# ColumbiaDVMM/ColumbiaImageSearch

Measured on AMD Instinct MI355X. Metric: queries/sec @ recall@10 on 10M LOPQ index, higher is better.
Workload: dtype f64

## Files before the change

### __graft_entry__.py

```python
import os
import subprocess
import sys

REPO = os.path.dirname(os.path.abspath(__file__))
if REPO not in sys.path:
    sys.path.insert(0, REPO)


def build():
    csrc = os.path.join(REPO, "columbiaimagesearch_amd", "csrc")
    subprocess.check_call(["make", "-C", csrc, "-j4"])
    from columbiaimagesearch_amd import _lib
    import columbiaimagesearch_amd.lopq
    assert _lib.lib().cis_version() >= 100


def smoke():
    import numpy as np
    sys.path.insert(0, os.path.join(REPO, "tests"))
    from conftest import load_golden
    from test_lopq_hip_parity import hip_model
    from columbiaimagesearch_amd.lopq import LOPQSearcherHIP
    from oracle import lopq_oracle as O
    z, X, Q = load_golden("c2")
    m = hip_model(z)
    n = 20000
    coarse, fine = m.predict_batch(X[:n])
    om = O.OracleModel.from_npz(z)
    oc, of = O.compute_codes(om, X[:n])
    assert (coarse == oc).all() and (fine == of).all(), "encode parity"
    s = LOPQSearcherHIP(m)
    s.add_codes_array(coarse, fine)
    oi = O.OracleCSRIndex(om, oc, of)
    want = [oi.search(Q[qi], quota=1000, limit=100) for qi in range(16)]
    for route, prefilter in (("float32-prefilter scan", True), ("all-candidates select", False)):
        s.set_scan_mode(prefilter_only=prefilter)
        r = s.search_batch(Q[:16], quota=1000, limit=100)
        for qi in range(16):
            ids, dists, visited = want[qi]
            k = int(r["n_found"][qi])
            assert k == len(ids) and visited == int(r["visited"][qi]), "visited / count parity (%s)" % route
            assert (r["ids"][qi, :k] == ids).all(), "candidate id parity (%s)" % route
            assert np.allclose(r["dists"][qi, :k], dists, rtol=1e-9, atol=1e-12), "distance parity (%s)" % route
    print("smoke ok: %d vectors encoded, 16 queries searched on both routes, parity with oracle" % n)


if __name__ == "__main__":
    build()
    if len(sys.argv) > 1 and sys.argv[1] == "smoke":
        smoke()
```

### columbiaimagesearch_amd/csrc/lopq_search.hip

```cpp
#include "lopq_batch.h"

template <typename CT>
__global__ __launch_bounds__(256) void k_tables(const CT* __restrict__ X , const CT* __restrict__ Cs,
                                                const double* __restrict__ Rt, const double* __restrict__ mus,
                                                const double* __restrict__ subs, const TabDesc* __restrict__ tabs,
                                                int V, int h, int w, int nf, int K, int D,
                                                double* __restrict__ T , PwProg prog_w,
                                                double* __restrict__ px_out ,
                                                const int* __restrict__ tab_order, int first) {
    extern __shared__ __attribute__((aligned(16))) char smem[];
    double* v = reinterpret_cast<double*>(smem);
    double* px = v + h;
    const int tab = tab_order ? tab_order[first + blockIdx.x] : first + (int)blockIdx.x;
    const TabDesc td = tabs[tab];
    const int s = td.split, c = td.cluster;
    const CT* x = X + (int64_t)td.q * D + s * h;
    const CT* Cc = Cs + ((int64_t)s * V + c) * h;
    const double* mu = mus + ((int64_t)s * V + c) * h;
    const double* R = Rt + ((int64_t)s * V + c) * h * h;
    for (int k = threadIdx.x; k < h; k += blockDim.x) {
        const CT res = x[k] - Cc[k];
        v[k] = (double)res - mu[k];
    }
    __syncthreads();
// ... 958 lines not shown
    constexpr double EPS32 = 2.0 * M * 5.9604644775390625e-8;
    const double infl = 1.0 + 2.0 * EPS32;
    CodeWords<M> dup[G];
    bool has_dup[G];
    bool any_dup = false;
#pragma unroll
    for (int g = 0; g < G; ++g) { cnt[g] = 0; has_dup[g] = false; dup[g] = CodeWords<M>(); }
#ifndef CIS_SCAN_PLAIN_LOADS
    __amdgpu_buffer_rsrc_t rs;
    {
        const uint64_t cbase = (uint64_t)(uintptr_t)(codes + start * M);
        const uint32_t blo = (uint32_t)__builtin_amdgcn_readfirstlane((int)(uint32_t)cbase);
        const uint32_t bhi = (uint32_t)__builtin_amdgcn_readfirstlane((int)(uint32_t)(cbase >> 32));
        const int nbytes = __builtin_amdgcn_readfirstlane(len * M);
        rs = __builtin_amdgcn_make_buffer_rsrc((void*)(uintptr_t)(((uint64_t)bhi << 32) | blo), 0, nbytes, 0x00020000);
    }
#define CIS_LOAD_CODE(p) load_code_buf<M>(rs, (p))
#else
#define CIS_LOAD_CODE(p) load_code<M>(codes, start + ((p) < len ? (p) : len - 1))
#endif
    CodeWords<M> nxt[U];
    if (w < nit) {
#pragma unroll
        for (int u = 0; u < U; ++u) nxt[u] = CIS_LOAD_CODE(w * 64 * U + u * 64 + lane);
    }
    for (int iter = w; iter < nit; iter += NW) {
        const int base = iter * 64 * U;
        CodeWords<M> cur[U];
#pragma unroll
        for (int u = 0; u < U; ++u) cur[u] = nxt[u];
        if (iter + NW < nit) {
#pragma unroll
            for (int u = 0; u < U; ++u) nxt[u] = CIS_LOAD_CODE((iter + NW) * 64 * U + u * 64 + lane);
        }
        float d[U][G];
#ifndef CIS_SCAN_NO_PIPELINE
        if constexpr (G >= 2) {
            typename AdcVec<G>::type fbuf[2][M];
            adc32_issue<M, G>(cur[0], tab, rc, fbuf[0]);
#pragma unroll
            for (int u = 0; u < U; ++u) {
                if (u + 1 < U) adc32_issue<M, G>(cur[u + 1], tab, rc, fbuf[(u + 1) & 1]);
                __builtin_amdgcn_sched_barrier(0);
                adc32_reduce<M, G>(fbuf[u & 1], d[u]);
                __builtin_amdgcn_sched_barrier(0);
            }
        } else
#endif
        {
#pragma unroll
            for (int u = 0; u < U; ++u) adc32g<M, G>(cur[u], tab, rc, d[u]);
        }
        if (base + 64 * U > len) {
            const float QNAN = __int_as_float(0x7fc00000);
#pragma unroll
            for (int u = 0; u < U; ++u)
#pragma unroll
                for (int g = 0; g < G; ++g) d[u][g] = (base + u * 64 + lane < len) ? d[u][g] : QNAN;
        }
        unsigned long long pm[U][G];
        unsigned long long any = 0ull;
#pragma unroll
        for (int g = 0; g < G; ++g) {
            float thrm = block_bound_f32(&sh[g]) * margin;
#ifdef CIS_PROBE_HOTLOOP
            thrm = (margin > 100.f) ? thrm : -1.0f;
#endif
#pragma unroll
            for (int u = 0; u < U; ++u) {
                pm[u][g] = __ballot(d[u][g] <= thrm);
                any |= pm[u][g];
            }
        }
        if (any_dup) {
            any = 0ull;
#pragma unroll
            for (int g = 0; g < G; ++g) {
                const unsigned long long dup_on = has_dup[g] ? ~0ull : 0ull;
#pragma unroll
                for (int u = 0; u < U; ++u) {
                    bool same = true;
#pragma unroll
                    for (int i = 0; i < (M + 3) / 4; ++i) same = same && (cur[u].w[i] == dup[g].w[i]);
                    pm[u][g] &= ~(__ballot(same) & dup_on);
                    any |= pm[u][g];
                }
            }
        }
        if (any == 0ull) continue;
        const long long clk_s0 = CIS_CLK();
        ++n_slow;
#pragma unroll
        for (int g = 0; g < G; ++g) {
            if (g >= ng) break;
            uint64_t* rk = rk_all + (g * NW + w) * R;
            uint64_t* tr = tr_all + (g * NW + w) * 64;
            uint32_t* rp = nullptr;
            int ntot = 0;
#pragma unroll
            for (int u = 0; u < U; ++u) ntot += __popcll(pm[u][g]);
            if (ntot == 0) continue;
            if (cnt[g] + ntot <= R) {
                const int trash = (int)(tr - rk) + lane;
                int c = cnt[g];
#pragma unroll
                for (int u = 0; u < U; ++u) {
                    const unsigned long long m = pm[u][g];
                    const int idx = __builtin_amdgcn_mbcnt_hi((unsigned)(m >> 32), __builtin_amdgcn_mbcnt_lo((unsigned)m, c));
                    int sel;
                    asm("v_cndmask_b32_e64 %0, %1, %2, %3" : "=v"(sel) : "v"(trash), "v"(idx), "s"(m));
                    rk[sel] = ((uint64_t)__float_as_uint(d[u][g]) << 32) | (uint32_t)(base + u * 64 + lane);
                    c += __popcll(m);
                }
                cnt[g] = c;
                n_app += ntot;
                continue;
            }
            int u0 = 0;
            while (true) {
                bool full = false;
#pragma unroll
                for (int u = 0; u < U; ++u) {
                    const unsigned long long m = pm[u][g];
                    if (u < u0 || full || m == 0ull) continue;
                    const int n = __popcll(m);
                    if (cnt[g] + n > R) {
                        full = true;
                        u0 = u;
                        continue;
                    }
                    const int idx = cnt[g] + __builtin_amdgcn_mbcnt_hi((unsigned)(m >> 32), __builtin_amdgcn_mbcnt_lo((unsigned)m, 0));
                    if ((m >> lane) & 1ull) rk[idx] = ((uint64_t)__float_as_uint(d[u][g]) << 32) | (uint32_t)(base + u * 64 + lane);
                    cnt[g] += n;
                    n_app += n;
                    u0 = u + 1;
                }
                if (!full) break;
                const long long clk_c0 = CIS_CLK();
                int c2 = wave_compact_approx<NR, NW>(rk, cnt[g], L, Lw, R - 64, margin, infl, &sh[g], w);
                if (c2 < 0) {
                    uint32_t dp = 0xffffffffu;
                    const long long clk_e0 = CIS_CLK();
                    c2 = wave_compact_exact<M, NR, NW, false>(rk, rp, cnt[g], L, Lw, &sh[g], w, codes, start, K, T + (int64_t)it_tab0[g] * nf * K,
                                                                  T + (int64_t)it_tab1[g] * nf * K, dp);
                    clk_exact += CIS_CLK() - clk_e0;
                    dp = (uint32_t)__builtin_amdgcn_readfirstlane((int)dp);
                    if (dp != 0xffffffffu) {
                        dup[g] = load_code<M>(codes, start + (int64_t)dp);
                        has_dup[g] = true;
                        any_dup = true;
                    }
                }
                cnt[g] = c2;
                clk_comp += CIS_CLK() - clk_c0;
                const float thrm = block_bound_f32(&sh[g]) * margin;
                const unsigned long long dup_on = has_dup[g] ? ~0ull : 0ull;
#pragma unroll
                for (int u = 0; u < U; ++u) {
                    bool same = true;
#pragma unroll
                    for (int i = 0; i < (M + 3) / 4; ++i) same = same && (cur[u].w[i] == dup[g].w[i]);
                    pm[u][g] &= __ballot(d[u][g] <= thrm) & ~(__ballot(same) & dup_on);
                }
            }
        }
        clk_slow += CIS_CLK() - clk_s0;
    }
    const long long clk_loop_end = CIS_CLK();
    (void)clk_loop_end;
#pragma unroll
    for (int g = 0; g < G; ++g) {
        if (g >= ng) break;
        uint64_t* rk = rk_all + (g * NW + w) * R;
        if (cnt[g] > 0) cnt[g] = wave_compact_approx<NR, NW>(rk, cnt[g], L, Lw, NR * 64, margin, infl, &sh[g], w);
    }
    clk_final = CIS_CLK() - clk_loop_end;
    __syncthreads();
#pragma unroll
    for (int g = 0; g < G; ++g) {
        if (g >= ng) break;
        uint64_t* rk = rk_all + (g * NW + w) * R;
        cnt[g] = wave_filter_approx<NR, NW>(rk, cnt[g], margin, &sh[g]);
        if (lane == 0) sh[g].wcnt[w] = cnt[g];
#ifndef CIS_SCAN_NO_QBOUND
        if (tid == 0) {
            const uint64_t b = block_bound_u64<NW>(&sh[g]);
            if (b < sh[g].ext) atomicMin(&qbound[it_q[g]], (unsigned long long)b);
        }
#endif
    }
    const long long clk_exact_end = CIS_CLK();
    (void)clk_exact_end;
    __syncthreads();
#pragma unroll
    for (int g = 0; g < G; ++g) {
        if (g >= ng) break;
        const uint64_t* rk = rk_all + (g * NW + w) * R;
        int off = 0, total = 0;
#pragma unroll
        for (int i = 0; i < NW; ++i) {
            const int c = sh[g].wcnt[i];
            off += (i < w) ? c : 0;
            total += c;
        }
        uint64_t* out = item_surv + (int64_t)item_idx[g] * S + off;
        for (int e = lane; e < cnt[g]; e += 64) out[e] = rk[e];
        if (tid == 0) item_n[item_idx[g]] = total;
    }
#ifdef CIS_SCAN_COUNTERS
    CIS_CTR(3, n_slow);
    CIS_CTR(8, clk_exact);
    CIS_CTR(10, clk_exact_end - clk_loop_end);
    CIS_CTR(11, clk_tab_end - clk_begin);
    CIS_CTR(9, clk_final);
    CIS_CTR(4, n_app);
    CIS_CTR(5, clk_comp);
    CIS_CTR(6, clk_slow - clk_comp);
    CIS_CTR(7, CIS_CLK() - clk_begin);
    CIS_CTR(2, clk_loop_end - clk_begin);
#endif
}

template <int M, int NR, int U, int G, int NW>
__global__ __launch_bounds__(NW * 64) __attribute__((amdgpu_waves_per_eu(NR == 16 ? 2 : (G == 4 ? 2 : ((M == 16 && G == 2) ? 3 : 4)), 4))) void k_adc_scan2(const WorkItem* __restrict__ items, const int* __restrict__ slots,
                                                       const int* __restrict__ n_slots_ptr, const double* __restrict__ T,
                                                       const float* __restrict__ T32,
                                                       const uint8_t* __restrict__ codes, const int64_t* __restrict__ ids,
                                                       int K, int L, int S, float margin,
                                                       int* __restrict__ queue_ctr ,
                                                       uint64_t* __restrict__ item_surv, int* __restrict__ item_n,
                                                       unsigned long long* __restrict__ qbound ) {
    extern __shared__ __attribute__((aligned(16))) char smem[];
    constexpr int R = NR * 64 - 8;
    int* s_next = reinterpret_cast<int*>(smem + (size_t)K * M * G * 4 + (size_t)G * NW * (R + 64) * 8 + G * sizeof(ScanShared));
    const int* qs = n_slots_ptr + 8;
    const int home = blockIdx.x & 7;
    for (int a = 0; a < 8; ++a) {
        const int x = (home + a) & 7;
        const int qstart = qs[x];
        const int count = qs[x + 1] - qstart;
        while (true) {
            __syncthreads();
            if (threadIdx.x == 0) *s_next = atomicAdd(&queue_ctr[x], 1);
            __syncthreads();
            const int j = __builtin_amdgcn_readfirstlane(*s_next);
            if (j >= count) break;
            const int slot = qstart + j;
            int idx[G];
            int ng = 0;
            bool same = true;
#pragma unroll
            for (int g = 0; g < G; ++g) {
                idx[g] = slots[slot * G + g];
                if (idx[g] >= 0) {
                    ng = g + 1;
                    same = same && items[idx[g]].start == items[idx[0]].start && items[idx[g]].len == items[idx[0]].len;
                } else {
                    idx[g] = idx[0];
                }
            }
            if constexpr (G >= 2) {
                if (!same) {
                    for (int g2 = 0; g2 < ng; ++g2) {
                        int oi[G];
#pragma unroll
                        for (int g = 0; g < G; ++g) {
                            oi[g] = idx[0];
#pragma unroll
                            for (int gg = 1; gg < G; ++gg)
                                if (gg == g2) oi[g] = idx[gg];
                        }
                        if (g2 > 0) __syncthreads();
                        scan2_group<M, NR, U, G, NW>(items, oi, 1, T, T32, codes, ids, K, L, S, margin, item_surv, item_n, qbound, smem);
                    }
                    continue;
                }
            }
            scan2_group<M, NR, U, G, NW>(items, idx, ng, T, T32, codes, ids, K, L, S, margin, item_surv, item_n, qbound, smem);
        }
    }
}

template <int CAPM>
__global__ __launch_bounds__(256) void k_merge_items(const cis_hit* __restrict__ item_hits, const int* __restrict__ item_n,
                                                     const int64_t* __restrict__ item_off, int limit, int S,
                                                     cis_hit* __restrict__ out_hits, int64_t* __restrict__ out_ids,
                                                     double* __restrict__ out_dists, int* __restrict__ out_n,
                                                     int32_t* __restrict__ out_cells, uint32_t* __restrict__ out_pos) {
    extern __shared__ __attribute__((aligned(16))) char smem[];
    uint64_t* ka = reinterpret_cast<uint64_t*>(smem);
    uint64_t* kb = ka + CAPM;
    int64_t* pay = reinterpret_cast<int64_t*>(kb + CAPM);
    int* s_n = reinterpret_cast<int*>(pay + CAPM);
    const int q = blockIdx.x;
    const int64_t a = item_off[q], b = item_off[q + 1];
    const int64_t o = (int64_t)q * limit;
    merge_lists<CAPM>(item_hits, item_n, a, (int)(b - a), (int64_t)S, S, limit, ka, kb, pay, s_n,
                      out_hits ? out_hits + o : nullptr, out_ids ? out_ids + o : nullptr,
                      out_dists ? out_dists + o : nullptr, out_n ? out_n + q : nullptr,
                      out_cells ? out_cells + o : nullptr, out_pos ? out_pos + o : nullptr);
}


static __device__ __forceinline__ void wave_bitonic_lds(uint64_t* ka, uint64_t* kb, int N) {
    const int lane = threadIdx.x & 63;
    for (int k = 2; k <= N; k <<= 1) {
        for (int j = k >> 1; j > 0; j >>= 1) {
            for (int t = lane; t < (N >> 1); t += 64) {
                const int i = ((t & ~(j - 1)) << 1) | (t & (j - 1));
                const int p = i + j;
                const bool asc = ((i & k) == 0);
                const uint64_t a0 = ka[i], b0 = kb[i], a1 = ka[p], b1 = kb[p];
                const bool gt = (a0 > a1) || (a0 == a1 && b0 > b1);
                if (gt == asc) { ka[i] = a1; kb[i] = b1; ka[p] = a0; kb[p] = b0; }
            }
            wave_lds_sync();
        }
    }
}

template <int CAPM, int MT , int NEMAX >
#ifndef CIS_MERGE_WPE
#define CIS_MERGE_WPE 4
#endif
__global__ __launch_bounds__(256) __attribute__((amdgpu_waves_per_eu((MT == 16 || MT == 0) ? 2 : CIS_MERGE_WPE, 8)))
void k_merge_survivors(const uint64_t* __restrict__ surv ,
                                                         const int* __restrict__ item_n, const int64_t* __restrict__ item_off,
                                                         const WorkItem* __restrict__ items, const double* __restrict__ T,
                                                         const uint8_t* __restrict__ codes, const int64_t* __restrict__ ids,
                                                         int nq, int M, int K, int limit, int S,
                                                         cis_hit* __restrict__ out_hits, int64_t* __restrict__ out_ids,
                                                         double* __restrict__ out_dists, int* __restrict__ out_n,
                                                         int32_t* __restrict__ out_cells, uint32_t* __restrict__ out_pos,
                                                         const PlanOut* __restrict__ plan, int32_t* __restrict__ out_visited,
                                                         const float* __restrict__ item_slack ) {
    extern __shared__ __attribute__((aligned(16))) char smem[];
    const int lane = threadIdx.x & 63, wq = threadIdx.x >> 6;
    const int q = blockIdx.x * 4 + wq;
    if (q >= nq) return;
    if (lane == 0 && out_visited) out_visited[q] = plan[q].visited;
    uint64_t* ka = reinterpret_cast<uint64_t*>(smem) + (size_t)wq * 2 * CAPM;
    uint64_t* kb = ka + CAPM;
    const int64_t first = item_off[q];
    const int n_lists = (int)(item_off[q + 1] - first);
    const int nf = M / 2;
    int have = 0, l = 0, e = 0, total = 0;
    bool done_fast = false;
    if constexpr (MT != 0) {
        int cntl[4] = {0, 0, 0, 0}, n_total = 0;
        if (n_lists <= 4) {
#pragma unroll
            for (int i = 0; i < 4; ++i) {
                if (i < n_lists) cntl[i] = item_n[first + i];
                n_total += cntl[i];
            }
        }
        auto fast = [&](auto ne_tag) -> bool {
            constexpr int NE = decltype(ne_tag)::value;
            uint32_t hi[NE], pp[NE];
            int li[NE];
            bool valid[NE];
            uint32_t mn = 0xffffffffu, mx = 0u;
            uint64_t ent[NE];
            float ubv[NE];
#pragma unroll
            for (int i = 0; i < NE; ++i) {
                const int x = lane + 64 * i;
                valid[i] = x < n_total;
                int lst = 0, off = x;
#pragma unroll
                for (int j = 0; j < 3; ++j)
                    if (lst == j && off >= cntl[j]) { off -= cntl[j]; lst = j + 1; }
                li[i] = lst;
                ent[i] = surv[valid[i] ? (first + lst) * (int64_t)S + off : first * (int64_t)S];
            }
            if (item_slack) {
#pragma unroll
                for (int i = 0; i < NE; ++i) ubv[i] = item_slack[2 * (first + (valid[i] ? li[i] : 0)) + 1];
            }
#pragma unroll
            for (int i = 0; i < NE; ++i) {
                hi[i] = valid[i] ? (uint32_t)(ent[i] >> 32) : 0xffffffffu;
                pp[i] = valid[i] ? (uint32_t)ent[i] : 0xffffffffu;
                if (item_slack && valid[i])
                    hi[i] = __float_as_uint(__double2float_ru((double)(hi[i] + (uint32_t)MT) * (double)ubv[i]));
                mn = (valid[i] && hi[i] < mn) ? hi[i] : mn;
                mx = (valid[i] && hi[i] > mx) ? hi[i] : mx;
            }
            uint32_t thr = 0xffffffffu;
            float vub = __int_as_float(0x7f800000);
            float sl[4] = {0.f, 0.f, 0.f, 0.f};
            if (n_total > limit) {
                wave_minmax_step<1>(mn, mx); wave_minmax_step<2>(mn, mx); wave_minmax_step<4>(mn, mx);
                wave_minmax_step<8>(mn, mx); wave_minmax_step<16>(mn, mx); wave_minmax_step<32>(mn, mx);
                mn = (uint32_t)__builtin_amdgcn_readfirstlane((int)mn);
                mx = (uint32_t)__builtin_amdgcn_readfirstlane((int)mx);
                const uint32_t v = wave_kth_bisect<NE>(hi, valid, mn, mx, limit);
                if (item_slack) {
                    vub = __uint_as_float(v);
#pragma unroll
                    for (int i = 0; i < 4; ++i) sl[i] = (i < n_lists) ? item_slack[2 * (first + i)] : 0.f;
                } else {
                    const float margin = 1.0f + 3.0f * (2.0f * (float)MT * 5.9604645e-8f);
                    thr = __float_as_uint(__double2float_ru((double)__uint_as_float(v) * (double)margin));
                }
            }
            int kept = 0;
            int idx[NE];
            bool keep[NE];
#pragma unroll
            for (int i = 0; i < NE; ++i) {
                keep[i] = valid[i] && hi[i] <= thr;
                if (item_slack) {
                    const float s_i = li[i] == 0 ? sl[0] : (li[i] == 1 ? sl[1] : (li[i] == 2 ? sl[2] : sl[3]));
                    keep[i] = valid[i] && ((double)__uint_as_float(hi[i]) - (double)s_i <= (double)vub);
                }
                const unsigned long long m = __ballot(keep[i]);
                idx[i] = kept + __builtin_amdgcn_mbcnt_hi((unsigned)(m >> 32), __builtin_amdgcn_mbcnt_lo((unsigned)m, 0));
                kept += __popcll(m);
            }
            if (kept > CAPM) return false;
            WorkItem its[4];
#pragma unroll
            for (int i = 0; i < 4; ++i) its[i] = items[first + (i < n_lists ? i : 0)];
#pragma unroll
            for (int i0 = 0; i0 < NE; i0 += 4) {
                int64_t startv[4];
                const double* t0v[4];
                const double* t1v[4];
                uint32_t rankv[4], pos0v[4];
#pragma unroll
                for (int i = 0; i < 4; ++i) {
                    WorkItem it = its[0];
#pragma unroll
                    for (int j = 1; j < 4; ++j)
                        if (li[i0 + i] == j) it = its[j];
                    startv[i] = it.start; rankv[i] = (uint32_t)it.rank; pos0v[i] = (uint32_t)it.pos0;
                    t0v[i] = T + (int64_t)it.tab0 * nf * K;
                    t1v[i] = T + (int64_t)it.tab1 * nf * K;
                }
                CodeWords<MT> cw[4];
#pragma unroll
                for (int i = 0; i < 4; ++i) cw[i] = load_code<MT>(codes, startv[i] + (keep[i0 + i] ? pp[i0 + i] : 0u));
                double dd[4];
#pragma unroll
                for (int i = 0; i < 4; ++i) dd[i] = adc64_words<MT>(cw[i].w, K, t0v[i], t1v[i]);
#pragma unroll
                for (int i = 0; i < 4; ++i) {
                    if (keep[i0 + i]) {
                        ka[idx[i0 + i]] = (uint64_t)__double_as_longlong(dd[i]);
                        kb[idx[i0 + i]] = ((uint64_t)rankv[i] << 32) | (uint32_t)(pos0v[i] + pp[i0 + i]);
                    }
                }
            }
            int ns = 64;
            while (ns < kept) ns <<= 1;
            for (int x = kept + lane; x < ns; x += 64) { ka[x] = ~0ull; kb[x] = ~0ull; }
            wave_lds_sync();
            wave_bitonic_lds(ka, kb, ns);
            total = kept;
            return true;
        };
        if (n_lists >= 1 && n_lists <= 4) {
            if (n_total <= 256) done_fast = fast(std::integral_constant<int, 4>());
            else if (NEMAX >= 8 && n_total <= 512) {
                if constexpr (NEMAX >= 8) done_fast = fast(std::integral_constant<int, 8>());
            }
        }
    }
    while (!done_fast) {
        int n = have;
        int room = CAPM - have;
        while (l < n_lists && room > 0) {
            const int valid = item_n[first + l];
            const int take = (valid - e < room) ? (valid - e) : room;
            if (take > 0) {
                const WorkItem it = items[first + l];
                const double* t0 = T + (int64_t)it.tab0 * nf * K;
                const double* t1 = T + (int64_t)it.tab1 * nf * K;
                const uint64_t* src = surv + (first + l) * (int64_t)S + e;
                if constexpr (MT == 0) {
                    for (int x = lane; x < take; x += 64) {
                        const uint32_t p = (uint32_t)src[x];
                        ka[n + x] = (uint64_t)__double_as_longlong(adc64_global(codes, it.start + p, M, K, t0, t1));
                        kb[n + x] = ((uint64_t)(uint32_t)it.rank << 32) | (uint32_t)(it.pos0 + (int)p);
                    }
                } else {
                    for (int x0 = 0; x0 < take; x0 += 256) {
                        uint32_t p[4];
                        bool on[4];
#pragma unroll
                        for (int i = 0; i < 4; ++i) {
                            const int x = x0 + i * 64 + lane;
                            on[i] = x < take;
                            p[i] = on[i] ? (uint32_t)src[x] : 0u;
                        }
                        CodeWords<MT> cw[4];
#pragma unroll
                        for (int i = 0; i < 4; ++i) cw[i] = load_code<MT>(codes, it.start + p[i]);
                        double dd[4];
#pragma unroll
                        for (int i = 0; i < 4; ++i) dd[i] = adc64_words<MT>(cw[i].w, K, t0, t1);
#pragma unroll
                        for (int i = 0; i < 4; ++i) {
                            const int x = x0 + i * 64 + lane;
                            if (on[i]) {
                                ka[n + x] = (uint64_t)__double_as_longlong(dd[i]);
                                kb[n + x] = ((uint64_t)(uint32_t)it.rank << 32) | (uint32_t)(it.pos0 + (int)p[i]);
                            }
                        }
                    }
                }
            }
            n += take;
            total += take;
            room -= take;
            e += take;
            if (e >= valid) { ++l; e = 0; }
        }
        int ns = 64;
        while (ns < n) ns <<= 1;
        for (int x = n + lane; x < ns; x += 64) { ka[x] = ~0ull; kb[x] = ~0ull; }
        wave_lds_sync();
        wave_bitonic_lds(ka, kb, ns);
        have = n < limit ? n : limit;
        if (l >= n_lists) break;
    }
    const int nv = total < limit ? total : limit;
    const int64_t o = (int64_t)q * limit;
    for (int x = lane; x < limit; x += 64) {
        cis_hit hh;
        hh.dist = __longlong_as_double(0x7ff0000000000000LL);
        hh.visit_rank = 0xffffffffu; hh.pos = 0xffffffffu; hh.id = -1; hh.cell = -1; hh.reserved = 0;
        if (x < nv) {
            const uint32_t rank = (uint32_t)(kb[x] >> 32), pos = (uint32_t)kb[x];
            for (int li = 0; li < n_lists; ++li) {
                const WorkItem it = items[first + li];
                const uint32_t rel = pos - (uint32_t)it.pos0;
                if ((uint32_t)it.rank == rank && rel < (uint32_t)it.len) {
                    hh.dist = __longlong_as_double((long long)ka[x]);
                    hh.visit_rank = rank;
                    hh.pos = pos;
                    hh.id = ids[it.start + rel];
                    hh.cell = it.cell;
                    break;
                }
            }
        }
        if (out_hits) out_hits[o + x] = hh;
        if (out_ids) {
            out_ids[o + x] = hh.id;
            out_dists[o + x] = (x < nv) ? hh.dist : __longlong_as_double(0x7ff8000000000000LL);
        }
        if (out_cells) out_cells[o + x] = hh.cell;
        if (out_pos) out_pos[o + x] = hh.pos;
    }
    if (lane == 0 && out_n) out_n[q] = nv;
}

__global__ void k_copy_visited(const PlanOut* __restrict__ plan, int nq, int32_t* __restrict__ visited) {
    const int q = blockIdx.x * blockDim.x + threadIdx.x;
    if (q < nq) visited[q] = plan[q].visited;
}


extern "C" int cis_index_set_profiling(cis_index* ix, int enable) {
    CIS_REQUIRE(ix != nullptr, "index is NULL");
    ix->profiling = enable < 0 ? 0 : (enable > 2 ? 2 : enable);
    return CIS_OK;
}

template <int LJ>
__device__ int selftest_xor(uint32_t v) { return lane_xor<LJ>(v) != (uint32_t)__shfl_xor((int)v, LJ) ? 1 : 0; }

template <int NR>
__device__ int selftest_sort(uint32_t seed) {
    const int lane = threadIdx.x & 63;
    uint32_t k[NR];
#pragma unroll
    for (int r = 0; r < NR; ++r) {
        uint32_t x = seed ^ (uint32_t)(lane * NR + r) * 2654435761u;
        x ^= x >> 15; x *= 2246822519u; x ^= x >> 13;
        k[r] = x % 1000u;
    }
    uint32_t mine[NR];
#pragma unroll
    for (int r = 0; r < NR; ++r) mine[r] = k[r];
    wave_bitonic_sort<NR>(k);
    int bad = 0;
#pragma unroll
    for (int r = 0; r + 1 < NR; ++r) bad += k[r] > k[r + 1];
    const uint32_t nxt = (uint32_t)__shfl_down((int)k[0], 1);
    if (lane < 63) bad += k[NR - 1] > nxt;
    uint32_t s0 = 0, s1 = 0, x0 = 0, x1 = 0;
#pragma unroll
    for (int r = 0; r < NR; ++r) { s0 += mine[r]; s1 += k[r]; x0 ^= mine[r] * 40503u; x1 ^= k[r] * 40503u; }
    for (int o = 32; o > 0; o >>= 1) {
        s0 += (uint32_t)__shfl_xor((int)s0, o); s1 += (uint32_t)__shfl_xor((int)s1, o);
        x0 ^= (uint32_t)__shfl_xor((int)x0, o); x1 ^= (uint32_t)__shfl_xor((int)x1, o);
    }
    bad += (s0 != s1) + (x0 != x1);
    return bad;
}

__global__ void k_selftest(int* __restrict__ errors) {
    const uint32_t v = (uint32_t)threadIdx.x * 7919u + blockIdx.x * 104729u + 17u;
    int bad = selftest_xor<1>(v) + selftest_xor<2>(v) + selftest_xor<4>(v) + selftest_xor<8>(v) + selftest_xor<16>(v) +
              selftest_xor<32>(v);
    bad += selftest_sort<4>(blockIdx.x * 977u + 1u) + selftest_sort<8>(blockIdx.x * 31u + 5u);
    if (bad) atomicAdd(errors, bad);
}

#ifdef CIS_SCAN_COUNTERS
extern "C" int cis_debug_counters(unsigned long long* out, int reset) {
    CIS_CHECK_HIP(hipMemcpyFromSymbol(out, HIP_SYMBOL(g_scan_ctr), 16 * sizeof(unsigned long long)));
    if (reset) {
        unsigned long long z[16] = {0};
        CIS_CHECK_HIP(hipMemcpyToSymbol(HIP_SYMBOL(g_scan_ctr), z, sizeof(z)));
    }
    return CIS_OK;
}
#endif

extern "C" int cis_selftest(int* n_errors) {
    CIS_REQUIRE(n_errors != nullptr, "NULL argument");
    CIS_TRY(cis_lazy_init());
    int* d = nullptr;
    CIS_CHECK_HIP(hipMalloc((void**)&d, sizeof(int)));
    CIS_CHECK_HIP(hipMemset(d, 0, sizeof(int)));
    hipLaunchKernelGGL(k_selftest, dim3(64), dim3(64), 0, nullptr, d);
    CIS_CHECK_HIP(hipMemcpy(n_errors, d, sizeof(int), hipMemcpyDeviceToHost));
    (void)hipFree(d);
    return CIS_OK;
}

extern "C" int cis_index_set_scan_mode(cis_index* ix, int mode) {
    CIS_REQUIRE(ix != nullptr && mode >= 0 && mode <= 7, "bad scan mode");
    ix->force_stream = (mode == 6);
    ix->force_scan5 = (mode == 7);
    ix->force_exact_scan = (mode == 1);
    ix->force_prefilter_scan = (mode >= 2 && mode <= 5) || mode == 7;
    ix->force_scan2 = (mode == 2);
    ix->force_scan3 = (mode == 3 || mode == 4 || mode == 5 || mode == 7);
    ix->force_two_pass = mode == 3 ? 0 : (mode == 4 ? 1 : ((mode == 5 || mode == 7) ? 2 : -1));
    return CIS_OK;
}

extern "C" int cis_index_read_profile(cis_index* ix, double ms[5], int64_t* launches) {
    CIS_REQUIRE(ix != nullptr && ms != nullptr, "NULL argument");
    for (auto& r : ix->prof) {
        hipEvent_t last = r.ev[4] ? r.ev[4] : r.ev[3];
        if (last) CIS_CHECK_HIP(hipEventSynchronize(last));
        for (int i = 0; i < 4; ++i) {
            if (!r.ev[i] || !r.ev[i + 1]) continue;
            float t = 0.f;
            CIS_CHECK_HIP(hipEventElapsedTime(&t, r.ev[i], r.ev[i + 1]));
            ix->prof_ms[i] += t;
        }
        if (r.has_scan && r.ev[5] && r.ev[3]) {
            float t = 0.f;
            CIS_CHECK_HIP(hipEventElapsedTime(&t, r.ev[5], r.ev[3]));
            ix->prof_ms[4] += t;
            ix->prof_launches += 1;
        }
        for (int i = 0; i < 6; ++i)
            if (r.ev[i]) (void)hipEventDestroy(r.ev[i]);
    }
    ix->prof.clear();
    for (int i = 0; i < 5; ++i) { ms[i] = ix->prof_ms[i]; ix->prof_ms[i] = 0; }
    if (launches) *launches = ix->prof_launches;
    ix->prof_launches = 0;
    return CIS_OK;
}

extern "C" int cis_index_last_scan_kernel(cis_index* ix) { return ix ? ix->last_scan_kernel : 0; }

extern "C" int cis_index_stream_counters(cis_index* ix, int64_t counters[2]) {
    CIS_REQUIRE(ix != nullptr && counters != nullptr, "NULL argument");
    counters[0] = ix->stream_batches;
    counters[1] = ix->stream_fallbacks;
    return CIS_OK;
}

extern "C" int cis_index_last_stats(cis_index* ix, int64_t stats[4]) {
    CIS_REQUIRE(ix != nullptr && stats != nullptr, "NULL argument");
    if (ix->stats_pending_seq) {
        if (__atomic_load_n(&ix->h_totals[3], __ATOMIC_ACQUIRE) != ix->stats_pending_seq) CIS_CHECK_HIP(hipDeviceSynchronize());
        ix->stats[0] += ix->h_totals[2];
        ix->stats[1] += ix->h_totals[0];
        ix->stats[2] += ix->h_totals[1];
        ix->stats_pending_seq = 0;
    }
    for (int i = 0; i < 4; ++i) stats[i] = ix->stats[i];
    return CIS_OK;
}

template <int CAP, int U>
static void launch_scan_m(int M, const ScanArgs& a, int S, const int* flag) {
    const size_t lds = (size_t)CAP * 16 + (size_t)M * a.K * sizeof(double) + 16;
    dispatch_int<0, 4, 8, 16>((M == 4 || M == 8 || M == 16) ? M : 0, [&](auto m) {
        hipLaunchKernelGGL((k_adc_scan<decltype(m)::value, CAP, U>), dim3((unsigned)a.n_items), dim3(256), lds, a.st, a.items, a.T, a.codes, a.ids, M, a.K, a.L, S, flag,
                           reinterpret_cast<cis_hit*>(a.hits), a.hitn);
    });
}

static void launch_scan_exact(int M, const ScanArgs& a, int S, const int* flag) {
    if (a.L <= 512) launch_scan_m<1024, 2>(M, a, S, flag);
    else if (a.L <= 1024) launch_scan_m<2048, 4>(M, a, S, flag);
    else launch_scan_m<4096, 4>(M, a, S, flag);
}

static const int SCAN2_MAX_LIMIT = 952;
static bool scan2_supported(int M, int K, int L) {
    return (M == 4 || M == 8 || M == 16) && K <= 256 && K % 4 == 0 && L >= 1 && L <= SCAN2_MAX_LIMIT;
}

static Scan2Geom scan2_geom(int M, int K, int L, int nq) {
    Scan2Geom g;
    const int NR = (L <= 184) ? 4 : (L <= 440 ? 8 : 16);
    g.G = (nq >= 64 && NR < 16) ? 2 : 1;
    g.NW = 4;
    g.U = (g.G == 2) ? 4 : 2;
    if (const char* e = getenv("CIS_SCAN_GEOM")) {
        int a = 0, b = 0, c = 0;
        if (NR < 16 && sscanf(e, "%d,%d,%d", &a, &b, &c) == 3 && ((a == 1 && b == 4) || (a == 2 && b == 4) || (a == 2 && b == 8 && c == 2) || (a == 2 && (b == 1 || b == 2) && c == 4) || (a == 4 && b == 4 && c == 4 && NR == 4)) && (c == 2 || c == 4)) {
            g.G = a; g.NW = b; g.U = c;
        }
    }
    g.S = g.NW * (NR * 64 - 8);
    g.lds = (size_t)K * M * g.G * 4 + (size_t)g.G * g.NW * (NR * 64 - 8 + 64) * 8 + g.G * sizeof(ScanShared) + 16;
    return g;
}

template <int M, int NR, int G, int NW, int U>
static void launch_scan2_t(const Scan2Geom& g, const ScanArgs& a) {
    const float eps = 2.0f * (float)M * 5.9604645e-8f;
    const float margin = 1.0f + 3.0f * eps;
    const int per_cu = (int)(163840 / g.lds) < (32 / NW) ? (int)(163840 / g.lds) : (32 / NW);
    hipLaunchKernelGGL((k_adc_scan2<M, NR, U, G, NW>), dim3(persistent_grid(a, G, per_cu)), dim3(NW * 64), g.lds, a.st, a.items, a.slots, a.n_slots, a.T, a.T32, a.codes, a.ids,
                       a.K, a.L, g.S, margin, a.qctr, a.hits, a.hitn, a.qbound);
}

template <int M, int NR>
static void launch_scan2_mr(const Scan2Geom& g, const ScanArgs& a) {
#define CIS_SCAN2_CASE(GG, WW, UU) if (g.G == GG && g.NW == WW && g.U == UU) return launch_scan2_t<M, NR, GG, WW, UU>(g, a);
    CIS_SCAN2_CASE(1, 4, 2)
    if constexpr (NR != 16) {
        CIS_SCAN2_CASE(1, 4, 4)
        CIS_SCAN2_CASE(2, 4, 4)
        CIS_SCAN2_CASE(2, 4, 2)
        CIS_SCAN2_CASE(2, 8, 2)
        CIS_SCAN2_CASE(2, 1, 4)
        CIS_SCAN2_CASE(2, 2, 4)
    }
    if constexpr (NR == 4) { CIS_SCAN2_CASE(4, 4, 4) }
#undef CIS_SCAN2_CASE
}

static void launch_scan2(int M, const Scan2Geom& g, const ScanArgs& a) {
    dispatch_int<4, 8, 16>(M, [&](auto m) { dispatch_nr<16>(a.L, [&](auto nr) { launch_scan2_mr<decltype(m)::value, decltype(nr)::value>(g, a); }); });
}

int cis_seg_sort_u64(void* temp, size_t* temp_bytes, const uint64_t* keys_in, uint64_t* keys_out, const uint64_t* vals_in,
                     uint64_t* vals_out, int64_t n, int nseg, const int64_t* seg_begin, const int64_t* seg_end, hipStream_t st);

__global__ void k_item_lens(const WorkItem* __restrict__ items, int64_t n, int64_t* __restrict__ lens) {
    const int64_t i = (int64_t)blockIdx.x * blockDim.x + threadIdx.x;
    if (i < n) lens[i] = items[i].len;
}

__global__ void k_seg_begin(const int64_t* __restrict__ cand_start, const int64_t* __restrict__ item_off, int nq, int64_t n_items,
                            int64_t n_cand, int64_t* __restrict__ seg, unsigned long long* __restrict__ qmin,
                            unsigned long long* __restrict__ qmax) {
    const int q = blockIdx.x * blockDim.x + threadIdx.x;
    if (q > nq) return;
    const int64_t it = item_off[q];
    seg[q] = (q == nq || it >= n_items) ? n_cand : cand_start[it];
    if (qmin && q < nq) { qmin[q] = ~0ull; qmax[q] = 0ull; }
}

static const int CAND_TILE = 4096;
__global__ __launch_bounds__(256) void k_cand_tile_sum(const WorkItem* __restrict__ items, int64_t n_items, int64_t* __restrict__ tile_sums) {
    __shared__ int64_t s_w[4];
    const int64_t base = (int64_t)blockIdx.x * CAND_TILE;
    int64_t sum = 0;
    for (int e = threadIdx.x; e < CAND_TILE; e += 256)
        if (base + e < n_items) sum += items[base + e].len;
#pragma unroll
    for (int o = 32; o > 0; o >>= 1) sum += __shfl_xor(sum, o);
    if ((threadIdx.x & 63) == 0) s_w[threadIdx.x >> 6] = sum;
    __syncthreads();
    if (threadIdx.x == 0) tile_sums[blockIdx.x] = s_w[0] + s_w[1] + s_w[2] + s_w[3];
}

__global__ __launch_bounds__(1024) void k_cand_tile_scan(int64_t* __restrict__ tile_sums, int64_t ntiles) {
    __shared__ int64_t s_w[16];
    const int tid = threadIdx.x, lane = tid & 63, wv = tid >> 6;
    int64_t carry = 0;
    for (int64_t b0 = 0; b0 < ntiles; b0 += 1024) {
        const int64_t i = b0 + tid;
        const int64_t v = i < ntiles ? tile_sums[i] : 0;
        int64_t x = v;
#pragma unroll
        for (int d = 1; d < 64; d <<= 1) {
            const int64_t y = __shfl_up(x, d);
            if (lane >= d) x += y;
        }
        __syncthreads();
        if (lane == 63) s_w[wv] = x;
        __syncthreads();
        int64_t base = carry, tot = 0;
        for (int w = 0; w < 16; ++w) { if (w < wv) base += s_w[w]; tot += s_w[w]; }
        if (i < ntiles) tile_sums[i] = base + x - v;
        carry += tot;
    }
}

__global__ __launch_bounds__(256) void k_cand_tile_apply(const WorkItem* __restrict__ items, int64_t n_items,
                                                         const int64_t* __restrict__ tile_off, int64_t* __restrict__ cand_start) {
    __shared__ int64_t s_w[4];
    const int tid = threadIdx.x, lane = tid & 63, wv = tid >> 6;
    const int64_t base = (int64_t)blockIdx.x * CAND_TILE;
    int64_t carry = tile_off[blockIdx.x];
    for (int e0 = 0; e0 < CAND_TILE; e0 += 256) {
        const int64_t i = base + e0 + tid;
        const int64_t v = i < n_items ? items[i].len : 0;
        int64_t x = v;
#pragma unroll
        for (int d = 1; d < 64; d <<= 1) {
            const int64_t y = __shfl_up(x, d);
            if (lane >= d) x += y;
        }
        __syncthreads();
        if (lane == 63) s_w[wv] = x;
        __syncthreads();
        int64_t b = carry;
        for (int w = 0; w < wv; ++w) b += s_w[w];
        if (i < n_items) cand_start[i] = b + x - v;
        carry += s_w[0] + s_w[1] + s_w[2] + s_w[3];
    }
}

__global__ __launch_bounds__(1024) void k_cand_layout(const WorkItem* __restrict__ items, int64_t n_items, const int64_t* __restrict__ item_off,
                                                      int nq, int64_t n_cand, int64_t* cand_start, int64_t* __restrict__ seg,
                                                      unsigned long long* __restrict__ qmin, unsigned long long* __restrict__ qmax,
                                                      const int64_t* __restrict__ d_totals ) {
    __shared__ int64_t s_w[16];
    if (d_totals) { n_items = d_totals[0]; n_cand = d_totals[2]; }
    const int tid = threadIdx.x, lane = tid & 63, wv = tid >> 6;
// ... 1743 lines not shown
```

Measured before the change: 22.82 million.

## Sort small merge sets in registers and reuse preloaded work items

```diff
diff --git a/__graft_entry__.py b/__graft_entry__.py
--- a/__graft_entry__.py
+++ b/__graft_entry__.py
@@ -9,7 +9,7 @@
 
 def build():
     csrc = os.path.join(REPO, "columbiaimagesearch_amd", "csrc")
-    subprocess.check_call(["make", "-C", csrc, "-j4"])
+    subprocess.check_call(["make", "-C", csrc, "-j4", "all", "counters"])
     from columbiaimagesearch_amd import _lib
     import columbiaimagesearch_amd.lopq
     assert _lib.lib().cis_version() >= 100
diff --git a/columbiaimagesearch_amd/csrc/lopq_search.hip b/columbiaimagesearch_amd/csrc/lopq_search.hip
--- a/columbiaimagesearch_amd/csrc/lopq_search.hip
+++ b/columbiaimagesearch_amd/csrc/lopq_search.hip
@@ -1284,6 +1284,27 @@
 }
 
 
+#ifdef CIS_MERGE_COUNTERS
+__device__ unsigned long long g_merge_ctr[32];
+#define CIS_MCTR(i, v) do { if ((threadIdx.x & 63) == 0) atomicAdd(&g_merge_ctr[i], (unsigned long long)(v)); } while (0)
+extern "C" int cis_debug_merge_counters(unsigned long long* out, int reset) {
+    CIS_CHECK_HIP(hipDeviceSynchronize());
+    CIS_CHECK_HIP(hipMemcpyFromSymbol(out, HIP_SYMBOL(g_merge_ctr), 32 * sizeof(unsigned long long)));
+    if (reset) {
+        unsigned long long z[32] = {0};
+        CIS_CHECK_HIP(hipMemcpyToSymbol(HIP_SYMBOL(g_merge_ctr), z, sizeof(z)));
+    }
+    return CIS_OK;
+}
+#else
+#define CIS_MCTR(i, v) do { } while (0)
+#endif
+static __device__ __forceinline__ int merge_bucket(int n, int first_cap, int n_buckets) {
+    int b = 0;
+    while (b < n_buckets - 1 && n > (first_cap << b)) ++b;
+    return b;
+}
+
 static __device__ __forceinline__ void wave_bitonic_lds(uint64_t* ka, uint64_t* kb, int N) {
     const int lane = threadIdx.x & 63;
     for (int k = 2; k <= N; k <<= 1) {
@@ -1299,6 +1320,64 @@
             wave_lds_sync();
         }
     }
+}
+
+template <int LJ>
+static __device__ __forceinline__ uint64_t lane_xor64(uint64_t v) {
+    return ((uint64_t)lane_xor<LJ>((uint32_t)(v >> 32)) << 32) | lane_xor<LJ>((uint32_t)v);
+}
+
+template <int NR, int KK, int J>
+static __device__ __forceinline__ void bitonic_step128(uint64_t (&a)[NR], uint64_t (&b)[NR]) {
+    const int lane = threadIdx.x & 63;
+    if constexpr (J < NR) {
+#pragma unroll
+        for (int r = 0; r < NR; ++r) {
+            if ((r & J) == 0) {
+                const bool asc = (((lane * NR + r) & KK) == 0);
+                const uint64_t a0 = a[r], b0 = b[r], a1 = a[r | J], b1 = b[r | J];
+                const bool gt = (a0 > a1) || (a0 == a1 && b0 > b1);
+                const bool sw = (gt == asc);
+                a[r] = sw ? a1 : a0; b[r] = sw ? b1 : b0;
+                a[r | J] = sw ? a0 : a1; b[r | J] = sw ? b0 : b1;
+            }
+        }
+    } else {
+        constexpr int LJ = J / NR;
+        const bool want_min = (((lane & LJ) == 0) == (((lane * NR) & KK) == 0));
+#pragma unroll
+        for (int r = 0; r < NR; ++r) {
+            const uint64_t oa = lane_xor64<LJ>(a[r]), ob = lane_xor64<LJ>(b[r]);
+            const bool gt = (a[r] > oa) || (a[r] == oa && b[r] > ob);
+            const bool take = (gt == want_min);
+            a[r] = take ? oa : a[r];
+            b[r] = take ? ob : b[r];
+        }
+    }
+}
+
+template <int NR, int KK, int J>
+static __device__ __forceinline__ void bitonic_merge128(uint64_t (&a)[NR], uint64_t (&b)[NR]) {
+    bitonic_step128<NR, KK, J>(a, b);
+    if constexpr (J > 1) bitonic_merge128<NR, KK, J / 2>(a, b);
+}
+
+template <int NR, int KK>
+static __device__ __forceinline__ void bitonic_levels128(uint64_t (&a)[NR], uint64_t (&b)[NR]) {
+    if constexpr (KK > 2) bitonic_levels128<NR, KK / 2>(a, b);
+    bitonic_merge128<NR, KK, KK / 2>(a, b);
+}
+
+template <int NR>
+static __device__ __forceinline__ void wave_bitonic_regs(uint64_t* ka, uint64_t* kb) {
+    const int lane = threadIdx.x & 63;
+    uint64_t a[NR], b[NR];
+#pragma unroll
+    for (int r = 0; r < NR; ++r) { a[r] = ka[lane * NR + r]; b[r] = kb[lane * NR + r]; }
+    bitonic_levels128<NR, NR * 64>(a, b);
+#pragma unroll
+    for (int r = 0; r < NR; ++r) { ka[lane * NR + r] = a[r]; kb[lane * NR + r] = b[r]; }
+    wave_lds_sync();
 }
 
 template <int CAPM, int MT , int NEMAX >
@@ -1318,7 +1397,7 @@
                                                          const float* __restrict__ item_slack ) {
     extern __shared__ __attribute__((aligned(16))) char smem[];
     const int lane = threadIdx.x & 63, wq = threadIdx.x >> 6;
-    const int q = blockIdx.x * 4 + wq;
+    const int q = __builtin_amdgcn_readfirstlane((int)(blockIdx.x * 4 + wq));
     if (q >= nq) return;
     if (lane == 0 && out_visited) out_visited[q] = plan[q].visited;
     uint64_t* ka = reinterpret_cast<uint64_t*>(smem) + (size_t)wq * 2 * CAPM;
@@ -1328,6 +1407,21 @@
     const int nf = M / 2;
     int have = 0, l = 0, e = 0, total = 0;
     bool done_fast = false;
+    const bool few_lists = MT != 0 && n_lists >= 1 && n_lists <= 4;
+    WorkItem its[4] = {};
+    if (few_lists) {
+#pragma unroll
+        for (int i = 0; i < 4; ++i) its[i] = items[first + (i < n_lists ? i : 0)];
+    }
+#ifdef CIS_MERGE_COUNTERS
+    {
+        int nt = 0;
+        for (int i = 0; i < n_lists; ++i) nt += item_n[first + i];
+        CIS_MCTR(24, 1);
+        CIS_MCTR(n_lists < 5 ? n_lists : 5, 1);
+        CIS_MCTR(6 + merge_bucket(nt, 64, 6), 1);
+    }
+#endif
     if constexpr (MT != 0) {
         int cntl[4] = {0, 0, 0, 0}, n_total = 0;
         if (n_lists <= 4) {
@@ -1401,10 +1495,9 @@
                 idx[i] = kept + __builtin_amdgcn_mbcnt_hi((unsigned)(m >> 32), __builtin_amdgcn_mbcnt_lo((unsigned)m, 0));
                 kept += __popcll(m);
             }
-            if (kept > CAPM) return false;
-            WorkItem its[4];
-#pragma unroll
-            for (int i = 0; i < 4; ++i) its[i] = items[first + (i < n_lists ? i : 0)];
+            if (kept > CAPM) { CIS_MCTR(21, 1); return false; }
+            CIS_MCTR(NE == 4 ? 17 : (NE == 8 ? 18 : 19), 1);
+            CIS_MCTR(23, kept);
 #pragma unroll
             for (int i0 = 0; i0 < NE; i0 += 4) {
                 int64_t startv[4];
@@ -1438,8 +1531,11 @@
             int ns = 64;
             while (ns < kept) ns <<= 1;
             for (int x = kept + lane; x < ns; x += 64) { ka[x] = ~0ull; kb[x] = ~0ull; }
+            CIS_MCTR(12 + merge_bucket(ns, 64, 5), 1);
             wave_lds_sync();
-            wave_bitonic_lds(ka, kb, ns);
+            if (ns == 64) wave_bitonic_regs<1>(ka, kb);
+            else if (ns == 128) wave_bitonic_regs<2>(ka, kb);
+            else wave_bitonic_lds(ka, kb, ns);
             total = kept;
             return true;
         };
@@ -1450,7 +1546,9 @@
             }
         }
     }
+    if (!done_fast) CIS_MCTR(20, 1);
     while (!done_fast) {
+        CIS_MCTR(22, 1);
         int n = have;
         int room = CAPM - have;
         while (l < n_lists && room > 0) {
@@ -1494,6 +1592,7 @@
                     }
                 }
             }
+            CIS_MCTR(23, take);
             n += take;
             total += take;
             room -= take;
@@ -1516,17 +1615,31 @@
         hh.visit_rank = 0xffffffffu; hh.pos = 0xffffffffu; hh.id = -1; hh.cell = -1; hh.reserved = 0;
         if (x < nv) {
             const uint32_t rank = (uint32_t)(kb[x] >> 32), pos = (uint32_t)kb[x];
-            for (int li = 0; li < n_lists; ++li) {
-                const WorkItem it = items[first + li];
+            auto from_item = [&](const WorkItem& it) -> bool {
                 const uint32_t rel = pos - (uint32_t)it.pos0;
-                if ((uint32_t)it.rank == rank && rel < (uint32_t)it.len) {
-                    hh.dist = __longlong_as_double((long long)ka[x]);
-                    hh.visit_rank = rank;
-                    hh.pos = pos;
-                    hh.id = ids[it.start + rel];
-                    hh.cell = it.cell;
-                    break;
+                if ((uint32_t)it.rank != rank || rel >= (uint32_t)it.len) return false;
+                hh.dist = __longlong_as_double((long long)ka[x]);
+                hh.visit_rank = rank;
+                hh.pos = pos;
+                hh.id = ids[it.start + rel];
+                hh.cell = it.cell;
+                return true;
+            };
+            if (few_lists) {
+                int li = -1;
+#pragma unroll
+                for (int j = 3; j >= 0; --j) {
+                    const uint32_t rel = pos - (uint32_t)its[j].pos0;
+                    if (j < n_lists && (uint32_t)its[j].rank == rank && rel < (uint32_t)its[j].len) li = j;
                 }
+                WorkItem it = its[0];
+#pragma unroll
+                for (int j = 1; j < 4; ++j)
+                    if (li == j) it = its[j];
+                if (li >= 0) from_item(it);
+            } else {
+                for (int li = 0; li < n_lists; ++li)
+                    if (from_item(items[first + li])) break;
             }
         }
         if (out_hits) out_hits[o + x] = hh;
```

Result: faster. 23.12 million, median of 4 (+1.3%).
